# Fancomi2017/InstanceFusion

Hardware: AMD Instinct MI355X
Metric: frames/s + ms/frame (ICP|fuse|instance) at 640x480, 5M surfels, 1/2/4/8 GPU (higher is better)
Workload: dtype f32; 1 GPU; 5000000-surfel map, 640x480 synthetic RGBD stream, 3-level ICP+RGB + surfel fuse + canned-mask instance votes with superpixel refinement; surfels_live=4734799, surfel_slots=4734799, map_order=random, parallelism=replicas x1, loop_frames=90

## Files before the change

instancefusion_amd/csrc/ifx_ctx.h:

```cpp
#pragma once
#include <hip/hip_runtime.h>
#include <stdint.h>
#include <string>
#include <vector>
#include <map>
#include "../../include/ifx_c_api.h"
#include "ifx_dev.h"

#ifndef IFX_LIST_SEGS
#define IFX_LIST_SEGS 8
#endif

struct DevState {
    float pose[16];
    float pose_inv[16];
    float last_pose[16];
    float weighting;
    int dense_enough;
    int count;
    int n_dead;
    int n_new;
    int overflow;
    unsigned int r_max_bits;
    float Rprev[9], tprev[3], Rprev_inv[9];
    float Rcurr[9], tcurr[3];
    double resultRt[16];
    float krkinv[9], kt[3];
    double resultR[9], lastResultR[9];
    float R_lr[9];
    float so3_lastError, so3_lastCount;
    int so3_done;
    float imageBasis[9], kinv[9], krlr[9];
    float lastICPError, lastICPCount, lastRGBError, lastRGBCount, lastSO3Error, lastSO3Count;
    double lastA[36], lastb[6];
    float icp29[29], rgb29[29];
    int rgb_count, rgb_sigma;
    int seg_counts[2];
    int seg_acc[2];
    int fold_total;
    alignas(64) int fold_acc[16][4];
    int first_live;
    int app_count0; unsigned int app_seq0, app_vln0;
    unsigned int result_ticket;
    unsigned int next_seq;
    int hot_stale;
    int range_exceeded;
    float spec_pose[16], spec_pose_inv[16], spec_weighting;
    int skip;
    float lc[24];
    int lc_candidates;
    float vl_pose[16];
    int vl_valid;
    int vl_scan;
    int vl_age;
    int vl_scans;
    unsigned int vl_n[2];
    unsigned int vl_seg_n[2 * IFX_LIST_SEGS], vl_seg_off[2 * IFX_LIST_SEGS];
    long long dbg[8];
    alignas(64) int gn_res[2];
    unsigned int gn_ticket;
    int gn_pad[13];
    double gn_acc[2 * IFX_ACC_REPL * IFX_ACC_STRIDE];
    double gn_acc2[2 * 2 * IFX_ACC_REPL * IFX_ACC_STRIDE];
    alignas(64) int gn_res2[2 * 16];
    alignas(64) unsigned int gn_bar[4 * 32 * 16];
    int gn_timeout;
    int gn_abort;
    int gn_done_seq;
    int gn_spin_limit, gn_fault;
    alignas(64) double gnp_acc[2 * 2 * IFX_ACC_REPL * IFX_ACC_STRIDE];
    alignas(64) int gnp_res[2 * 16];
    alignas(64) double gnp_RRt[2][16];
};

struct IdMap { const uint32_t* seq; int own_n; };
__device__ __forceinline__ int idmap_slot(const IdMap& m, int count, int id)
{
    if (m.own_n <= 0) return (id > 0 && id < count) ? id : -1;
    if (id == 0) return -1;
    int lo = 0, hi = count - 1;
    while (lo <= hi) {
        const int mid = (lo + hi) >> 1;
        const unsigned int v = m.seq[mid];
        if (v == (unsigned int)id) return mid;
        if (v < (unsigned int)id) lo = mid + 1; else hi = mid - 1;
    }
    return -1;
}

struct FrameResult {
// ... 428 lines not shown
```

instancefusion_amd/csrc/ifx_map.hip:

```cpp
#include <climits>
#include "ifx_ctx.h"
#include <string.h>

#define DEAD_TIME (-1.0e9f)
#define ASSOC_NONE 0xFFFFFFFFu
#define ASSOC_NEW 0xFFFFFFFEu
#define MAP_THREADS 256
#ifndef MAP_BLOCKS
#define MAP_BLOCKS 2048
#endif
#ifndef LIST_BLOCKS
#define LIST_BLOCKS 1024
#endif

__device__ inline float get_radius(float depth, float norm_z, float inv_fx, float inv_fy)
{
    float meanFocal = ((1.0f / fabsf(inv_fx)) + (1.0f / fabsf(inv_fy))) / 2.0f;
    const float sqrt2 = 1.41421356237f;
    float radius = (depth / meanFocal) * sqrt2;
    float radius_n = radius / fabsf(norm_z);
    radius_n = fminf(2.0f * radius, radius_n);
    return radius_n;
}
__device__ inline float confidence_fn(float x, float y, float cx, float cy, float weighting)
// ... 1318 lines not shown
        if (T < (float)c.age_epoch) return false;
    }
    return T - wv > 20.f;
}
__global__ void k_vlist_decide(DevState* st, unsigned int* lctr, int force)
{
    if (threadIdx.x != 0) return;
    if (force) st->vl_valid = 0;
    vlist_decide(st);
}

struct VlPlanes { float lx, lz, rx, rz, ty, tz, by, bz; };
__device__ __forceinline__ bool near_frustum(v3 q, float reach, const VlPlanes& P, float maxDepth)
{
    const float len = sqrtf(q.x * q.x + q.y * q.y + q.z * q.z);
    const float D = (reach + VL_TRANS + VL_ROT * (len + reach + VL_TRANS)) * 1.01f + 0.01f;
    if (!(len == len)) return true;
    return !(P.lx * q.x + P.lz * q.z > D || P.rx * q.x + P.rz * q.z > D || P.ty * q.y + P.tz * q.z > D || P.by * q.y + P.bz * q.z > D || -q.z > D || q.z - maxDepth > D);
}
static VlPlanes make_planes(const Cam& c)
{
    VlPlanes P;
    float n = sqrtf(c.fx * c.fx + c.cx * c.cx);
    P.lx = -c.fx / n; P.lz = -c.cx / n;
    n = sqrtf(c.fx * c.fx + (c.cx - c.w) * (c.cx - c.w));
    P.rx = c.fx / n; P.rz = (c.cx - c.w) / n;
    n = sqrtf(c.fy * c.fy + c.cy * c.cy);
    P.ty = -c.fy / n; P.tz = -c.cy / n;
    n = sqrtf(c.fy * c.fy + (c.cy - c.h) * (c.cy - c.h));
    P.by = c.fy / n; P.bz = (c.cy - c.h) / n;
    return P;
}

__global__ __launch_bounds__(MAP_THREADS) void k_cull_frame(DevState* st, const float4* __restrict__ pc_in, float4* __restrict__ pc_rw, float2* __restrict__ tm, Cam c, VlPlanes P,
                                                            int time, unsigned int* __restrict__ list, unsigned int* __restrict__ list_i, Hot* __restrict__ hot, int time_prev)
{
    if (!st->vl_scan) return;
    float Tm[16], T[12];
#pragma unroll
    for (int k = 0; k < 16; k++) Tm[k] = st->vl_pose[k];
    {
        float inv[16];
        pose_inverse(Tm, inv);
#pragma unroll
        for (int k = 0; k < 12; k++) T[k] = inv[k];
    }
    __shared__ BlockCount2 L2;
    if (threadIdx.x == 0) { L2.n[0] = 0; L2.n[1] = 0; }
    __syncthreads();
    const int n = st->count;
    const float reach = __uint_as_float(st->r_max_bits) * 1.41421356f * 1.001f;
    int dead = 0;
    constexpr int CF_ROUNDS = 8, CF_SLOTS = MAP_THREADS * CF_ROUNDS;
    for (int chunk = blockIdx.x; chunk * CF_SLOTS < n; chunk += gridDim.x) {
        unsigned int pos[CF_ROUNDS];
        unsigned int keep = 0, keep_i = 0;
        float4 p4s[CF_ROUNDS];
        float2 ts[CF_ROUNDS];
#pragma unroll
        for (int r = 0; r < CF_ROUNDS; r++) {
            const int i = chunk * CF_SLOTS + r * MAP_THREADS + threadIdx.x;
            const int ii = i < n ? i : n - 1;
            p4s[r] = ld_once(&pc_in[ii]);
            ts[r] = ld_once(&tm[ii]);
        }
        asm volatile("" ::"v"(p4s[0].x), "v"(p4s[1].x), "v"(p4s[2].x), "v"(p4s[3].x), "v"(p4s[4].x), "v"(p4s[5].x), "v"(p4s[6].x), "v"(p4s[7].x), "v"(ts[0].x), "v"(ts[1].x), "v"(ts[2].x),
                     "v"(ts[3].x), "v"(ts[4].x), "v"(ts[5].x), "v"(ts[6].x), "v"(ts[7].x));
#pragma unroll
        for (int r = 0; r < CF_ROUNDS; r++) {
            const int i = chunk * CF_SLOTS + r * MAP_THREADS + threadIdx.x;
            bool in = false, in_i = false;
            if (i < n) {
                const float4 p4 = p4s[r];
                const float2 t = ts[r];
                const float wv = t.y;
                const bool overdue = age_rule_gone(wv, p4.w, time_prev, c) && wv > DEAD_TIME;
                if (overdue) {
                    float4 q4 = p4;
                    q4.w = -1.0f;
                    pc_rw[i] = q4;
                    tm[i] = make_float2(t.x, DEAD_TIME);
                    if (hot) { hot[i].pc = q4; hot[i].tm = make_float2(t.x, DEAD_TIME); }
                    dead++;
                } else if (wv > DEAD_TIME) {
                    in = near_frustum(xf_point(T, v3m(p4.x, p4.y, p4.z)), reach, P, c.maxDepth);
                    if (in && wv > 0.f && (float)time - wv > (float)c.timeDelta) {
                        in = false;
                        in_i = !(p4.w < c.conf);
                    }
                }
            }
            pos[r] = bcount2_reserve(L2, in, in_i);
            keep |= in ? (1u << r) : 0u;
            keep_i |= in_i ? (1u << r) : 0u;
        }
        __syncthreads();
        const int seg = chunk % LIST_SEGS;
        if (threadIdx.x < 2) { L2.base[threadIdx.x] = L2.n[threadIdx.x] ? atomicAdd(list_ctr(c, 1 + threadIdx.x, seg), L2.n[threadIdx.x]) : 0u; L2.n[threadIdx.x] = 0; }
        __syncthreads();
        const unsigned int ba = seg * c.seg_cap + L2.base[0], bi = seg * c.seg_cap + L2.base[1];
#pragma unroll
        for (int r = 0; r < CF_ROUNDS; r++) {
            const unsigned int i = (unsigned int)(chunk * CF_SLOTS + r * MAP_THREADS + threadIdx.x);
            if (keep & (1u << r)) list[ba + pos[r]] = i;
            if (keep_i & (1u << r)) list_i[bi + pos[r]] = i;
        }
    }
    dead = wave_sum_i(dead);
    if ((threadIdx.x & 63) == 0 && dead) atomicAdd(&st->n_dead, dead);
}

__global__ void k_vlist_offsets(DevState* st, Cam c, const float2* __restrict__ tm)
{
    if (!st->vl_scan || threadIdx.x != 0) return;
    for (int which = 0; which < 2; which++) {
        unsigned int run = 0;
        for (int seg = 0; seg < LIST_SEGS; seg++) {
            unsigned int* ctr = list_ctr(c, 1 + which, seg);
            const unsigned int n = *ctr;
            *ctr = 0;
            st->vl_seg_n[which * LIST_SEGS + seg] = n;
            st->vl_seg_off[which * LIST_SEGS + seg] = run;
            run += n;
        }
        st->vl_n[which] = run;
    }
    {
        int f = st->first_live;
        const int n = st->count;
        while (f < n && !(tm[f].y > DEAD_TIME)) f++;
        st->first_live = f;
    }
}
__global__ __launch_bounds__(MAP_THREADS) void k_vlist_concat(const DevState* __restrict__ st, Cam c, const unsigned int* __restrict__ raw_a, const unsigned int* __restrict__ raw_i,
                                                              unsigned int* __restrict__ flat_a, unsigned int* __restrict__ flat_i)
{
    if (!st->vl_scan) return;
    const int which = blockIdx.y, seg = blockIdx.x % LIST_SEGS;
    const unsigned int n = st->vl_seg_n[which * LIST_SEGS + seg], off = st->vl_seg_off[which * LIST_SEGS + seg];
    const unsigned int* __restrict__ raw = (which ? raw_i : raw_a) + (size_t)seg * c.seg_cap;
    unsigned int* __restrict__ flat = (which ? flat_i : flat_a) + off;
    for (unsigned int t = (blockIdx.x / LIST_SEGS) * blockDim.x + threadIdx.x; t < n; t += blockDim.x * (gridDim.x / LIST_SEGS)) flat[t] = raw[t];
}

__global__ __launch_bounds__(MAP_THREADS) void k_index_list(const DevState* __restrict__ st, const float4* __restrict__ pc, const float2* __restrict__ tm, Cam c, int time,
                                                            const unsigned int* __restrict__ list, unsigned long long* __restrict__ keys, const Hot* __restrict__ hot = nullptr)
{
    const int fl = FIRST_LIVE(c);
    float T[12];
#pragma unroll
    for (int k = 0; k < 12; k++) T[k] = st->pose_inv[k];
    const unsigned int n = min(st->vl_n[0], c.seg_cap * LIST_SEGS);
#ifndef INDEX_U
#define INDEX_U 1
#endif
    constexpr int U = INDEX_U;
    const unsigned int stride = blockDim.x * gridDim.x;
    for (unsigned int t = blockIdx.x * blockDim.x + threadIdx.x; t < n; t += U * stride) {
        unsigned int i[U];
        bool in[U];
#pragma unroll
        for (int u = 0; u < U; u++) { const unsigned int tt = t + u * stride; in[u] = tt < n; i[u] = list[in[u] ? tt : t]; }
        float lastT[U];
        float4 p4[U];
#pragma unroll
        for (int u = 0; u < U; u++) { lastT[u] = hot ? hot[i[u]].tm.y : ld_once(&tm[i[u]]).y; p4[u] = hot ? hot[i[u]].pc : ld_once(&pc[i[u]]); }
// ... 1110 lines not shown
{
    age_epoch_begin(h, time);
    h->hot_valid = 0;
    h->last_clean_time = time;
    Cam c = make_cam(h);
    if (part == 0) { c.srank = 0; c.sn = 1; }
    const bool deform = h->graph_nodes > 0 && part != 1;
    if (deform && !h->graph_is_fern) raster_pass(h, d_pose_inv, 0, time - h->cfg.time_delta, LIST_SPLAT, nullptr, false, 0, 1);
    if (part != 2) LAUNCH(h, "cull_clean", dim3(MAP_BLOCKS), dim3(MAP_THREADS), k_cull_clean, h->d_state, d_pose_inv, (const float4*)h->pc, (const float2*)h->tm, c, time, h->key_index,
           h->list_b, h->list_c);
    if (part == 1) return;
    launch_index_resolve(h, d_pose_inv, c, time, INDEX_TAPS, nullptr, nullptr);
    launch_clean_list(h, d_pose_inv, c, time);
    if (deform) {
        LAUNCH_SMEM(h, "deform", dim3(MAP_BLOCKS), dim3(256), (size_t)h->graph_nodes * 64, k_deform, h->d_state, d_pose_inv, h->d_graph, h->graph_nodes, h->graph_is_fern, time, c,
                    (const float4*)h->old_vertex, (float4*)h->pc, (float4*)h->nr, (float2*)h->tm);
        h->graph_nodes = 0;
    }
    launch_new_flags_count(h, d_pose_inv, c, time);
    launch_append_scan(h, c, time, h->own ? (unsigned int*)nullptr : h->list_v);
}

__global__ void k_vlist_invalidate(DevState* st) { if (threadIdx.x == 0) st->vl_valid = 0; }
void hs_invalidate_view(ifx* h) { h->ids_view_ok = 0; LAUNCH(h, "vlist_invalidate", dim3(1), dim3(64), k_vlist_invalidate, h->d_state); }
static void launch_vlist_decide(ifx* h, int force) { LAUNCH(h, "vlist_decide", dim3(1), dim3(64), k_vlist_decide, h->d_state, h->d_list_ctr, force); }
static bool use_view_list(ifx* h) { return h->opt_vlist && h->shard_n <= 1 && !h->own && !h->opt_reference_passes && h->graph_nodes == 0 && !h->view_block && h->tick > 1; }
static bool use_view_list_own(ifx* h) { return h->opt_vlist && h->own && !h->opt_reference_passes && h->graph_nodes == 0 && !h->view_block; }
static void view_scan(ifx* h, int time)
{
    const Cam c = whole_cam(h);
    LAUNCH(h, "cull_frame", dim3(MAP_BLOCKS), dim3(MAP_THREADS), k_cull_frame, h->d_state, (const float4*)h->pc, (float4*)h->pc, (float2*)h->tm, c, make_planes(c), time, h->list_b, h->list_c,
           h->hot_valid ? (Hot*)h->hot : (Hot*)nullptr,
           std::max(0, std::min(time, h->last_clean_time)));
    LAUNCH(h, "vlist_offsets", dim3(1), dim3(64), k_vlist_offsets, h->d_state, c, (const float2*)h->tm);
    LAUNCH(h, "vlist_concat", dim3(256, 2), dim3(MAP_THREADS), k_vlist_concat, (const DevState*)h->d_state, c, h->list_b, h->list_c, h->list_v, h->list_vi);
}
int ifx_vlist_reap(ifx* h)
{
    if (!h->view_dirty) return IFX_OK;
    h->view_dirty = 0;
    h->ids_view_ok = 0;
    launch_vlist_decide(h, 1);
    view_scan(h, h->last_clean_time);
    return IFX_OK;
}
static void index_list_pass(ifx* h, int time, bool taps)
{
    const Cam c = whole_cam(h);
    launch_index_list(h, c, time, (const Hot*)h->frame_hot);
    launch_index_resolve(h, nullptr, c, time, taps ? INDEX_TAPS : INDEX_ASSOC, nullptr, (const Hot*)h->frame_hot);
}

static void view_clean_append(ifx* h, const Cam& c, int time)
{
    h->hot_valid = 0;
    LAUNCH(h, "clean_view", dim3(h->opt_clean_blocks > 0 ? h->opt_clean_blocks : 2 * LIST_BLOCKS), dim3(MAP_THREADS), k_clean_view, h->d_state, c, time, (float4*)h->pc, (const float4*)h->nr, (float2*)h->tm,
           (const float4*)h->index_tap, h->list_v);
    launch_new_flags_count(h, nullptr, c, time);
    launch_append_scan(h, c, time, h->list_v);
}

int ifx_map_frame(ifx* h)
{
    h->clean_raster_pending = 0;
    h->view_frame = 0;
    h->ids_view_ok = 0;
    age_epoch_begin(h, h->tick);
// ... 592 lines not shown
```

instancefusion_amd/csrc/ifx_track.hip:

```cpp
#include "ifx_ctx.h"
#include <math.h>
#include <string.h>


#define BIL_R 6
#define BIL_BX 32
#define BIL_BY 8
template <bool SHIFTED, bool XCLIP>
__device__ __forceinline__ void bil_window(const uint16_t (*tile)[BIL_BX + 2 * BIL_R + 3], const unsigned char* s_mapx, const unsigned char* s_mapy, int x, int y, int bx, int by, int tx1,
                                           int ty1, unsigned int value, float& sum1, float& sum2)
{
    const float ss = 0.024691358f, sc = 0.000555556f;
    constexpr int D = BIL_R * 2 + 1;
    const float fv = (float)value;
    for (int cy = max(y - D / 2, 0); cy < ty1; ++cy) {
        const int ry = SHIFTED ? (int)s_mapy[cy - by + BIL_R + 1] : cy - by + BIL_R + 1;
        const float dy = (float)y - (float)cy, dy2 = dy * dy;
        float tv[D];
#pragma unroll
        for (int q = 0; q < D; q++) {
            const int col = x - D / 2 + q - bx + BIL_R + 1;
            tv[q] = (float)tile[ry][SHIFTED ? (int)s_mapx[col] : col];
        }
#pragma unroll
// ... 184 lines not shown
        v3 r = v3m(qn, qn, qn);
        if (!(u == w - 1 || v == h - 1) && ok00) {
            v3 v01, v10;
            bool ok01 = vert_from_depth(L.depth, w, u + 1, v, L.fx_inv, L.fy_inv, L.cx, L.cy, a.cutoff, v01);
            bool ok10 = vert_from_depth(L.depth, w, u, v + 1, L.fx_inv, L.fy_inv, L.cx, L.cy, a.cutoff, v10);
            if (ok01 && ok10) r = normalized(cross(v01 - v00, v10 - v00));
        }
        L.nmap[v * w + u] = r.x;
        L.nmap[(v + h) * w + u] = r.y;
        L.nmap[(v + 2 * h) * w + u] = r.z;
    }
    {
        const float gsx[9] = {0.52201f, 0.00000f, -0.52201f, 0.79451f, -0.00000f, -0.79451f, 0.52201f, 0.00000f, -0.52201f};
        const float gsy[9] = {0.52201f, 0.79451f, 0.52201f, 0.00000f, 0.00000f, 0.00000f, -0.52201f, -0.79451f, -0.52201f};
        float dxVal = 0, dyVal = 0;
        int k = 8;
        for (int j = max(v - 1, 0); j <= min(v + 1, h - 1); j++)
            for (int i = max(u - 1, 0); i <= min(u + 1, w - 1); i++) {
                dxVal += (float)L.img[j * w + i] * gsx[k];
                dyVal += (float)L.img[j * w + i] * gsy[k];
                --k;
            }
        L.dx[v * w + u] = (int16_t)dxVal;
        L.dy[v * w + u] = (int16_t)dyVal;
    }
}

struct ModelOut {
    float *vcam, *ncam, *depth;
    uint8_t* img;
    float *vprev, *nprev, *cloud;
    float invFx, invFy, cx, cy;
};
__device__ __forceinline__ void model_tail(const DevState* __restrict__ st, int x, int y, int w, int h, v3 vs, v3 ns, float z, const ModelOut& o)
{
    if (o.vprev) {
        const float* P = st->pose;
        const float qn = qnan_f();
        v3 vd = v3m(qn, qn, qn);
        if (!(vs.x != vs.x)) vd = xf_dir(P, vs) + v3m(P[3], P[7], P[11]);
        o.vprev[y * w + x] = vd.x; o.vprev[(y + h) * w + x] = vd.y; o.vprev[(y + 2 * h) * w + x] = vd.z;
        v3 nd = v3m(qn, qn, qn);
        if (!(ns.x != ns.x)) nd = xf_dir(P, ns);
        o.nprev[y * w + x] = nd.x; o.nprev[(y + h) * w + x] = nd.y; o.nprev[(y + 2 * h) * w + x] = nd.z;
    }
    if (o.cloud) {
        o.cloud[(y * w + x) * 3 + 0] = (float)((x - o.cx) * z * o.invFx);
        o.cloud[(y * w + x) * 3 + 1] = (float)((y - o.cy) * z * o.invFy);
        o.cloud[(y * w + x) * 3 + 2] = z;
    }
}
__global__ void k_model_l0(const DevState* __restrict__ st, const float* __restrict__ pv, const float* __restrict__ pn, const uint8_t* __restrict__ pi, const float* __restrict__ fv,
                           const float* __restrict__ fn, const uint8_t* __restrict__ fi, int w, int h, float cutoff, ModelOut o)
{
    int x = blockIdx.x * blockDim.x + threadIdx.x, y = blockIdx.y * blockDim.y + threadIdx.y;
    if (x >= w || y >= h) return;
    const bool fill = fv && !st->dense_enough;
    const float4 v = reinterpret_cast<const float4*>(fill ? fv : pv)[y * w + x];
    const float4 n = reinterpret_cast<const float4*>(fill ? fn : pn)[y * w + x];
    const uint8_t* s = (fill ? fi : pi) + (size_t)(y * w + x) * 4;
    const float qn = qnan_f();
    bool ok = !(v.z == 0);
    v3 vs = v3m(ok ? v.x : qn, ok ? v.y : qn, ok ? v.z : qn), ns = v3m(ok ? n.x : qn, ok ? n.y : qn, ok ? n.z : qn);
    o.vcam[y * w + x] = vs.x; o.vcam[(y + h) * w + x] = vs.y; o.vcam[(y + 2 * h) * w + x] = vs.z;
    o.ncam[y * w + x] = ns.x; o.ncam[(y + h) * w + x] = ns.y; o.ncam[(y + 2 * h) * w + x] = ns.z;
    const float z = (v.z > cutoff || v.z <= 0) ? qn : v.z;
    o.depth[y * w + x] = z;
    o.img[y * w + x] = (uint8_t)(int)((float)s[0] * 0.114f + (float)s[1] * 0.299f + (float)s[2] * 0.587f);
    model_tail(st, x, y, w, h, vs, ns, z, o);
}
struct GnBegin { DevState* st; const DevState* ss; int so3; float fx, fy, cx, cy; int keep_last, enabled, persist; };
__device__ void gn_begin_dev(DevState* st, const DevState* __restrict__ ss, int so3, float fx, float fy, float cx, float cy, int keep_last);
__device__ __forceinline__ void gn_persist_reset(DevState* st, int lt, int nt)
{
    for (int k = lt; k < 2 * 2 * IFX_ACC_REPL * IFX_ACC_STRIDE; k += nt) st->gn_acc2[k] = 0.0;
    if (lt < 32) st->gn_res2[lt] = 0;
    for (int k = lt; k < 4 * 32 * 16; k += nt) st->gn_bar[k] = 0u;
    if (lt == 0) { st->gn_abort = 0; st->gn_done_seq = 0; }
}
__global__ void k_model_down(const DevState* __restrict__ st, const float* __restrict__ vin, const float* __restrict__ nin, const float* __restrict__ din, const uint8_t* __restrict__ iin,
                             int sw, int sh, ModelOut o, GnBegin gb)
{
    if (gb.enabled && blockIdx.x == 0 && blockIdx.y == 0) {
        const int lt = threadIdx.y * blockDim.x + threadIdx.x, nt = blockDim.x * blockDim.y;
        if (gb.persist) gn_persist_reset(gb.st, lt, nt);
        if (lt == 0) gn_begin_dev(gb.st, gb.ss, gb.so3, gb.fx, gb.fy, gb.cx, gb.cy, gb.keep_last);
    }
    const int dw = sw / 2, dh = sh / 2;
    int x = blockIdx.x * blockDim.x + threadIdx.x, y = blockIdx.y * blockDim.y + threadIdx.y;
    if (x >= dw || y >= dh) return;
    const float qn = qnan_f();
    const int xs = x * 2, ys = y * 2;
    v3 res[2];
#pragma unroll
    for (int m = 0; m < 2; m++) {
        const float* in = m ? nin : vin;
        float* out = m ? o.ncam : o.vcam;
        float x00 = in[ys * sw + xs], x01 = in[ys * sw + xs + 1], x10 = in[(ys + 1) * sw + xs], x11 = in[(ys + 1) * sw + xs + 1];
        v3 n = v3m(qn, qn, qn);
        if (!((x00 != x00) || (x01 != x01) || (x10 != x10) || (x11 != x11))) {
            n.x = (x00 + x01 + x10 + x11) / 4;
            const float* py = in + sh * sw;
// ... 1705 lines not shown
                for (int k = 0; k < 9; k++) { st->Rcurr[k] = Rc[k]; st->krkinv[k] = krkn[k]; }
#pragma unroll
                for (int k = 0; k < 3; k++) { st->tcurr[k] = tcn[k]; st->kt[k] = ktn[k]; }
                if (a.final_level) track_end_vals(st, RGB, 1, Rc, tcn, Rp, tpv, a.weight_mult, a.commit, a.lctr);
                st->gn_done_seq = a.level + 1;
            }
        }
        __syncthreads();
    }
    (void)failed;
}


__global__ void k_commit_pose(DevState* st, unsigned int* lctr)
{
    (void)lctr;
    const int t = threadIdx.x;
    float cp = 0.f;
    if (t < 16) cp = st->spec_pose[t]; else if (t < 32) cp = st->spec_pose_inv[t - 16]; else if (t == 32) cp = st->spec_weighting;
    float A[16], B[16];
    int valid = 0, age = 0;
    if (t == 0) {
#pragma unroll
        for (int k = 0; k < 16; k++) { A[k] = st->vl_pose[k]; B[k] = st->spec_pose[k]; }
        valid = st->vl_valid; age = st->vl_age;
    }
    if (t < 16) st->pose[t] = cp; else if (t < 32) st->pose_inv[t - 16] = cp; else if (t == 32) st->weighting = cp;
    if (t != 0) return;
    vlist_decide_core(st, A, B, valid, age);
}



static const dim3 B2(32, 8);
static inline dim3 G2(int w, int h) { return dim3(cdiv(w, 32), cdiv(h, 8)); }

int ifx_alloc_tracker(ifx* h)
{
    Pyr& p = h->pyr;
    for (int i = 0; i < IFX_NUM_PYRS; i++) {
        p.w[i] = h->w >> i; p.h[i] = h->h >> i;
        size_t n = (size_t)p.w[i] * p.h[i];
        for (int q = 0; q < 2; q++) {
            FrameSlot& f = h->slot[q];
            HIPCHK(h, hipMalloc(&f.depth_tmp[i], n * 2));
            HIPCHK(h, hipMalloc(&f.vmap_curr[i], n * 12)); HIPCHK(h, hipMalloc(&f.nmap_curr[i], n * 12));
            HIPCHK(h, hipMalloc(&f.next_img[i], n)); HIPCHK(h, hipMemset(f.next_img[i], 0, n));
            HIPCHK(h, hipMalloc(&f.didx[i], n * 2)); HIPCHK(h, hipMalloc(&f.didy[i], n * 2));
        }
        HIPCHK(h, hipMalloc(&p.vmap_cam[i], n * 12)); HIPCHK(h, hipMalloc(&p.nmap_cam[i], n * 12));
        HIPCHK(h, hipMalloc(&p.vmap_prev[i], n * 12)); HIPCHK(h, hipMalloc(&p.nmap_prev[i], n * 12));
        HIPCHK(h, hipMalloc(&p.last_depth[i], n * 4));
        HIPCHK(h, hipMalloc(&p.last_img[i], n));
        HIPCHK(h, hipMalloc(&p.cloud[i], n * 12));
        HIPCHK(h, hipMalloc(&p.corres[i], n * 8));
    }
    const int maxb = 1024;
    HIPCHK(h, hipMalloc(&p.acc, (3 * IFX_ACC_REPL * IFX_ACC_STRIDE * sizeof(double))));
    HIPCHK(h, hipMemset(p.acc, 0, (3 * IFX_ACC_REPL * IFX_ACC_STRIDE * sizeof(double))));
    {
        int cus = 0, dev = 0;
        hipGetDevice(&dev);
        hipDeviceGetAttribute(&cus, hipDeviceAttributeMultiprocessorCount, dev);
        int occ[4] = {0, 0, 0, 0};
        hipOccupancyMaxActiveBlocksPerMultiprocessor(&occ[0], k_gn_level<1>, RED_THREADS, 0);
        hipOccupancyMaxActiveBlocksPerMultiprocessor(&occ[1], k_gn_level<2>, RED_THREADS, 0);
// ... 59 lines not shown
static inline int red_blocks(ifx* h, int n, int it = RED_IT)
{
    int b = cdiv(n, RED_THREADS * it);
    const int cap = h->opt_icp_blocks > 0 ? h->opt_icp_blocks : std::max(456, std::min(1024, h->P / 2048));
    if (b > cap) b = cap;
    if (b < 1) b = 1;
    return b;
}

int ifx_tracker_init_first(ifx* h)
{
    Pyr& p = h->pyr;
    LAUNCH(h, "intensity", dim3(cdiv(h->P, 256)), dim3(256), k_intensity, h->rgb, 3, h->P, p.lastnext_img[0]);
    for (int i = 0; i + 1 < IFX_NUM_PYRS; i++)
        LAUNCH(h, "pyrdown_u8", G2(p.w[i + 1], p.h[i + 1]), B2, k_pyrdown_gauss_u8, p.lastnext_img[i], p.w[i], p.h[i], p.lastnext_img[i + 1]);
    return IFX_OK;
}

static inline GnBegin gb_none() { GnBegin g; g.st = nullptr; g.ss = nullptr; g.so3 = 0; g.fx = g.fy = g.cx = g.cy = 0.f; g.keep_last = 0; g.enabled = 0; g.persist = 0; return g; }
static void tracker_init_model(ifx* h, DevState* st, Pyr& p, float icp_weight, const float* pv, const float* pn, const uint8_t* pi, const float* fv, const float* fn, const uint8_t* fi, const GnBegin* gbp = nullptr)
{
    const GnBegin gb_off = gb_none();
    const ifx_config& c = h->cfg;
    const int rgb = icp_weight < 100;
    const int iterations[3] = {c.fast_odom ? 3 : 10, c.pyramid ? 5 : 0, c.pyramid ? 4 : 0};
    ModelOut o3[IFX_NUM_PYRS];
    for (int i = 0; i < IFX_NUM_PYRS; i++) {
        const float div = (float)(1 << i);
        ModelOut& o = o3[i];
        o.vcam = p.vmap_cam[i]; o.ncam = p.nmap_cam[i]; o.depth = p.last_depth[i]; o.img = p.last_img[i];
        o.vprev = p.vmap_prev[i]; o.nprev = p.nmap_prev[i]; o.cloud = (rgb && iterations[i] > 0) ? p.cloud[i] : nullptr;
        o.invFx = 1.0f / (c.fx / div); o.invFy = 1.0f / (c.fy / div); o.cx = c.cx / div; o.cy = c.cy / div;
    }
    for (int i = 0; i < IFX_NUM_PYRS; i++) {
        const ModelOut& o = o3[i];
        if (i == 0) LAUNCH(h, "model_l0", G2(h->w, h->h), B2, k_model_l0, st, pv, pn, pi, fv, fn, fi, h->w, h->h, 6.0f, o);
        else LAUNCH(h, "model_down", G2(p.w[i], p.h[i]), B2, k_model_down, st, p.vmap_cam[i - 1], p.nmap_cam[i - 1], p.last_depth[i - 1], p.last_img[i - 1], p.w[i - 1], p.h[i - 1], o, (i == IFX_NUM_PYRS - 1 && gbp) ? *gbp : gb_off);
    }
}

__global__ void k_sobel(const uint8_t* __restrict__ img, int w, int h, int16_t* __restrict__ dx, int16_t* __restrict__ dy)
{
    const int u = blockIdx.x * blockDim.x + threadIdx.x, v = blockIdx.y * blockDim.y + threadIdx.y;
    if (u >= w || v >= h) return;
    const float gsx[9] = {0.52201f, 0.00000f, -0.52201f, 0.79451f, -0.00000f, -0.79451f, 0.52201f, 0.00000f, -0.52201f};
    const float gsy[9] = {0.52201f, 0.79451f, 0.52201f, 0.00000f, 0.00000f, 0.00000f, -0.52201f, -0.79451f, -0.52201f};
    float dxVal = 0, dyVal = 0;
    int k = 8;
    for (int j = max(v - 1, 0); j <= min(v + 1, h - 1); j++)
        for (int i = max(u - 1, 0); i <= min(u + 1, w - 1); i++) {
            dxVal += (float)img[j * w + i] * gsx[k];
            dyVal += (float)img[j * w + i] * gsy[k];
            --k;
        }
    dx[v * w + u] = (int16_t)dxVal;
    dy[v * w + u] = (int16_t)dyVal;
}
static void tracker_init_frame_maps(ifx* h, DevState* st, Pyr& p, const float* pv, const float* pn, const uint8_t* pi)
{
    for (int i = 0; i < IFX_NUM_PYRS; i++) {
        ModelOut o;
        o.vcam = p.vmap_curr[i]; o.ncam = p.nmap_curr[i]; o.depth = p.next_depth[i]; o.img = p.next_img[i];
        o.vprev = nullptr; o.nprev = nullptr; o.cloud = nullptr;
        o.invFx = 0; o.invFy = 0; o.cx = 0; o.cy = 0;
        if (i == 0) LAUNCH(h, "model_l0", G2(h->w, h->h), B2, k_model_l0, st, pv, pn, pi, (const float*)nullptr, (const float*)nullptr, (const uint8_t*)nullptr, h->w, h->h, 6.0f, o);
        else LAUNCH(h, "model_down", G2(p.w[i], p.h[i]), B2, k_model_down, st, p.vmap_curr[i - 1], p.nmap_curr[i - 1], p.next_depth[i - 1], p.next_img[i - 1], p.w[i - 1], p.h[i - 1], o, gb_none());
        LAUNCH(h, "sobel", G2(p.w[i], p.h[i]), B2, k_sobel, p.next_img[i], p.w[i], p.h[i], p.didx[i], p.didy[i]);
    }
}

static void tracker_init_frame(ifx* h, const uint16_t* depth_filt, const uint8_t* rgb)
{
    Pyr& p = h->pyr;
    (void)depth_filt;
    LAUNCH(h, "intensity", dim3(cdiv(h->P, 256)), dim3(256), k_intensity, rgb, 3, h->P, p.next_img[0]);
    for (int i = 1; i < IFX_NUM_PYRS; i++)
        LAUNCH(h, "frame_down", G2(p.w[i], p.h[i]), B2, k_frame_down, p.depth_tmp[i - 1], p.next_img[i - 1], p.w[i - 1], p.h[i - 1], p.depth_tmp[i], p.next_img[i]);
    FrameLevels fl;
    int blocks = 0;
    for (int i = 0; i < IFX_NUM_PYRS; i++) {
        float div = (float)(1 << i);
        float fx = h->cfg.fx / div, fy = h->cfg.fy / div;
        FrameLevel& L = fl.l[i];
        L.depth = p.depth_tmp[i]; L.img = p.next_img[i]; L.vmap = p.vmap_curr[i]; L.nmap = p.nmap_curr[i]; L.dx = p.didx[i]; L.dy = p.didy[i];
        L.w = p.w[i]; L.h = p.h[i]; L.tiles_x = cdiv(p.w[i], 32); L.first_block = blocks;
        L.fx_inv = 1.f / fx; L.fy_inv = 1.f / fy; L.cx = h->cfg.cx / div; L.cy = h->cfg.cy / div;
        blocks += L.tiles_x * cdiv(p.h[i], 8);
    }
    fl.cutoff = h->cfg.max_depth_processed;
    LAUNCH(h, "frame_maps", dim3(blocks), dim3(256), k_frame_maps, fl);
}

int ifx_comm_ready(ifx* h);
int ifx_comm_allreduce_f64(ifx* h, double* d_ptr, int n);
static inline const char* icp_name_rows(int level) { static const char* const n[3] = {"icp_residual_rows@L0", "icp_residual_rows@L1", "icp_residual_rows@L2"}; return n[level]; }
static void tracker_run(ifx* h, DevState* st, Pyr& p, float icp_weight, int so3, float weight_mult, int commit, bool frame_tracker, int keep_last = 0)
{
    const ifx_config& c = h->cfg;
    const int icp = icp_weight > 0, rgb = icp_weight < 100;
    int iterations[3] = {c.fast_odom ? 3 : 10, c.pyramid ? 5 : 0, c.pyramid ? 4 : 0};
    int first = -1;
// ... 703 lines not shown
```

Before: 1634 frames/s.

## Fuse vlist offsets into cull tail and merge model levels 0 and 1

Result: no change. 1643 frames/s (median of 4 runs) (+0.6%).

```diff
diff --git a/instancefusion_amd/csrc/ifx_ctx.h b/instancefusion_amd/csrc/ifx_ctx.h
--- a/instancefusion_amd/csrc/ifx_ctx.h
+++ b/instancefusion_amd/csrc/ifx_ctx.h
@@ -56,6 +56,8 @@
     int vl_scans;
     unsigned int vl_n[2];
     unsigned int vl_seg_n[2 * IFX_LIST_SEGS], vl_seg_off[2 * IFX_LIST_SEGS];
+    alignas(64) unsigned int vl_ticket;
+    int vl_pad[15];
     long long dbg[8];
     alignas(64) int gn_res[2];
     unsigned int gn_ticket;
diff --git a/instancefusion_amd/csrc/ifx_map.hip b/instancefusion_amd/csrc/ifx_map.hip
--- a/instancefusion_amd/csrc/ifx_map.hip
+++ b/instancefusion_amd/csrc/ifx_map.hip
@@ -1374,6 +1374,26 @@
     return P;
 }
 
+__device__ __forceinline__ void vlist_offsets_dev(DevState* st, const Cam& c, const float2* tm, int n)
+{
+    for (int which = 0; which < 2; which++) {
+        unsigned int run = 0;
+        for (int seg = 0; seg < LIST_SEGS; seg++) {
+            unsigned int* ctr = list_ctr(c, 1 + which, seg);
+            const unsigned int m = __hip_atomic_load(ctr, __ATOMIC_RELAXED, __HIP_MEMORY_SCOPE_AGENT);
+            __hip_atomic_store(ctr, 0u, __ATOMIC_RELAXED, __HIP_MEMORY_SCOPE_AGENT);
+            st->vl_seg_n[which * LIST_SEGS + seg] = m;
+            st->vl_seg_off[which * LIST_SEGS + seg] = run;
+            run += m;
+        }
+        st->vl_n[which] = run;
+    }
+    {
+        int f = st->first_live;
+        while (f < n && !(__hip_atomic_load(&tm[f].y, __ATOMIC_RELAXED, __HIP_MEMORY_SCOPE_AGENT) > DEAD_TIME)) f++;
+        st->first_live = f;
+    }
+}
 __global__ __launch_bounds__(MAP_THREADS) void k_cull_frame(DevState* st, const float4* __restrict__ pc_in, float4* __restrict__ pc_rw, float2* __restrict__ tm, Cam c, VlPlanes P,
                                                             int time, unsigned int* __restrict__ list, unsigned int* __restrict__ list_i, Hot* __restrict__ hot, int time_prev)
 {
@@ -1421,7 +1441,7 @@
                     float4 q4 = p4;
                     q4.w = -1.0f;
                     pc_rw[i] = q4;
-                    tm[i] = make_float2(t.x, DEAD_TIME);
+                    __hip_atomic_store(&tm[i].y, DEAD_TIME, __ATOMIC_RELAXED, __HIP_MEMORY_SCOPE_AGENT);
                     if (hot) { hot[i].pc = q4; hot[i].tm = make_float2(t.x, DEAD_TIME); }
                     dead++;
                 } else if (wv > DEAD_TIME) {
@@ -1450,30 +1470,19 @@
     }
     dead = wave_sum_i(dead);
     if ((threadIdx.x & 63) == 0 && dead) atomicAdd(&st->n_dead, dead);
-}
-
-__global__ void k_vlist_offsets(DevState* st, Cam c, const float2* __restrict__ tm)
-{
-    if (!st->vl_scan || threadIdx.x != 0) return;
-    for (int which = 0; which < 2; which++) {
-        unsigned int run = 0;
-        for (int seg = 0; seg < LIST_SEGS; seg++) {
-            unsigned int* ctr = list_ctr(c, 1 + which, seg);
-            const unsigned int n = *ctr;
-            *ctr = 0;
-            st->vl_seg_n[which * LIST_SEGS + seg] = n;
-            st->vl_seg_off[which * LIST_SEGS + seg] = run;
-            run += n;
-        }
-        st->vl_n[which] = run;
-    }
-    {
-        int f = st->first_live;
-        const int n = st->count;
-        while (f < n && !(tm[f].y > DEAD_TIME)) f++;
-        st->first_live = f;
-    }
-}
+    __shared__ int s_last;
+    asm volatile("s_waitcnt vmcnt(0)" ::: "memory");
+    __syncthreads();
+    if (threadIdx.x == 0) {
+        const unsigned int t = __hip_atomic_fetch_add(&st->vl_ticket, 1u, __ATOMIC_RELAXED, __HIP_MEMORY_SCOPE_AGENT);
+        s_last = (t == gridDim.x - 1u);
+    }
+    __syncthreads();
+    if (!s_last || threadIdx.x != 0) return;
+    __hip_atomic_store(&st->vl_ticket, 0u, __ATOMIC_RELAXED, __HIP_MEMORY_SCOPE_AGENT);
+    vlist_offsets_dev(st, c, tm, n);
+}
+
 __global__ __launch_bounds__(MAP_THREADS) void k_vlist_concat(const DevState* __restrict__ st, Cam c, const unsigned int* __restrict__ raw_a, const unsigned int* __restrict__ raw_i,
                                                               unsigned int* __restrict__ flat_a, unsigned int* __restrict__ flat_i)
 {
@@ -2650,7 +2659,6 @@
     LAUNCH(h, "cull_frame", dim3(MAP_BLOCKS), dim3(MAP_THREADS), k_cull_frame, h->d_state, (const float4*)h->pc, (float4*)h->pc, (float2*)h->tm, c, make_planes(c), time, h->list_b, h->list_c,
            h->hot_valid ? (Hot*)h->hot : (Hot*)nullptr,
            std::max(0, std::min(time, h->last_clean_time)));
-    LAUNCH(h, "vlist_offsets", dim3(1), dim3(64), k_vlist_offsets, h->d_state, c, (const float2*)h->tm);
     LAUNCH(h, "vlist_concat", dim3(256, 2), dim3(MAP_THREADS), k_vlist_concat, (const DevState*)h->d_state, c, h->list_b, h->list_c, h->list_v, h->list_vi);
 }
 int ifx_vlist_reap(ifx* h)
diff --git a/instancefusion_amd/csrc/ifx_track.hip b/instancefusion_amd/csrc/ifx_track.hip
--- a/instancefusion_amd/csrc/ifx_track.hip
+++ b/instancefusion_amd/csrc/ifx_track.hip
@@ -240,42 +240,131 @@
     float *vprev, *nprev, *cloud;
     float invFx, invFy, cx, cy;
 };
-__device__ __forceinline__ void model_tail(const DevState* __restrict__ st, int x, int y, int w, int h, v3 vs, v3 ns, float z, const ModelOut& o)
-{
+__device__ __forceinline__ void model_tail_vals(const DevState* __restrict__ st, int x, int y, v3 vs, v3 ns, float z, const ModelOut& o, v3& vd, v3& nd, v3& cl)
+{
+    const float qn = qnan_f();
+    vd = v3m(qn, qn, qn); nd = v3m(qn, qn, qn); cl = v3m(qn, qn, qn);
     if (o.vprev) {
         const float* P = st->pose;
-        const float qn = qnan_f();
-        v3 vd = v3m(qn, qn, qn);
         if (!(vs.x != vs.x)) vd = xf_dir(P, vs) + v3m(P[3], P[7], P[11]);
+        if (!(ns.x != ns.x)) nd = xf_dir(P, ns);
+    }
+    if (o.cloud) cl = v3m((float)((x - o.cx) * z * o.invFx), (float)((y - o.cy) * z * o.invFy), z);
+}
+__device__ __forceinline__ void model_tail(const DevState* __restrict__ st, int x, int y, int w, int h, v3 vs, v3 ns, float z, const ModelOut& o)
+{
+    v3 vd, nd, cl;
+    model_tail_vals(st, x, y, vs, ns, z, o, vd, nd, cl);
+    if (o.vprev) {
         o.vprev[y * w + x] = vd.x; o.vprev[(y + h) * w + x] = vd.y; o.vprev[(y + 2 * h) * w + x] = vd.z;
-        v3 nd = v3m(qn, qn, qn);
-        if (!(ns.x != ns.x)) nd = xf_dir(P, ns);
         o.nprev[y * w + x] = nd.x; o.nprev[(y + h) * w + x] = nd.y; o.nprev[(y + 2 * h) * w + x] = nd.z;
     }
     if (o.cloud) {
-        o.cloud[(y * w + x) * 3 + 0] = (float)((x - o.cx) * z * o.invFx);
-        o.cloud[(y * w + x) * 3 + 1] = (float)((y - o.cy) * z * o.invFy);
-        o.cloud[(y * w + x) * 3 + 2] = z;
-    }
-}
-__global__ void k_model_l0(const DevState* __restrict__ st, const float* __restrict__ pv, const float* __restrict__ pn, const uint8_t* __restrict__ pi, const float* __restrict__ fv,
-                           const float* __restrict__ fn, const uint8_t* __restrict__ fi, int w, int h, float cutoff, ModelOut o)
-{
-    int x = blockIdx.x * blockDim.x + threadIdx.x, y = blockIdx.y * blockDim.y + threadIdx.y;
-    if (x >= w || y >= h) return;
+        o.cloud[(y * w + x) * 3 + 0] = cl.x;
+        o.cloud[(y * w + x) * 3 + 1] = cl.y;
+        o.cloud[(y * w + x) * 3 + 2] = cl.z;
+    }
+}
+#define ML_TW 68
+#define ML_TH 20
+__device__ __forceinline__ void st_pair(float* p, float a, float b) { *reinterpret_cast<float2*>(p) = make_float2(a, b); }
+__global__ __launch_bounds__(256) void k_model_l0(const DevState* __restrict__ st, const float* __restrict__ pv, const float* __restrict__ pn, const uint8_t* __restrict__ pi,
+                                                   const float* __restrict__ fv, const float* __restrict__ fn, const uint8_t* __restrict__ fi, int w, int h, float cutoff, ModelOut o0,
+                                                   ModelOut o1)
+{
+    __shared__ float s_z[ML_TH][ML_TW];
+    __shared__ uint8_t s_i[ML_TH][ML_TW];
     const bool fill = fv && !st->dense_enough;
-    const float4 v = reinterpret_cast<const float4*>(fill ? fv : pv)[y * w + x];
-    const float4 n = reinterpret_cast<const float4*>(fill ? fn : pn)[y * w + x];
-    const uint8_t* s = (fill ? fi : pi) + (size_t)(y * w + x) * 4;
+    const float4* __restrict__ sv = reinterpret_cast<const float4*>(fill ? fv : pv);
+    const float4* __restrict__ sn = reinterpret_cast<const float4*>(fill ? fn : pn);
+    const uint8_t* __restrict__ si = fill ? fi : pi;
+    const int dw = w / 2, dh = h / 2;
+    const int x = blockIdx.x * 32 + threadIdx.x, y = blockIdx.y * 8 + threadIdx.y;
+    const int ox = blockIdx.x * 64 - 2, oy = blockIdx.y * 16 - 2;
     const float qn = qnan_f();
-    bool ok = !(v.z == 0);
-    v3 vs = v3m(ok ? v.x : qn, ok ? v.y : qn, ok ? v.z : qn), ns = v3m(ok ? n.x : qn, ok ? n.y : qn, ok ? n.z : qn);
-    o.vcam[y * w + x] = vs.x; o.vcam[(y + h) * w + x] = vs.y; o.vcam[(y + 2 * h) * w + x] = vs.z;
-    o.ncam[y * w + x] = ns.x; o.ncam[(y + h) * w + x] = ns.y; o.ncam[(y + 2 * h) * w + x] = ns.z;
-    const float z = (v.z > cutoff || v.z <= 0) ? qn : v.z;
-    o.depth[y * w + x] = z;
-    o.img[y * w + x] = (uint8_t)(int)((float)s[0] * 0.114f + (float)s[1] * 0.299f + (float)s[2] * 0.587f);
-    model_tail(st, x, y, w, h, vs, ns, z, o);
+    const bool mine = x < dw && y < dh;
+    v3 vs[2][2], ns[2][2];
+    if (mine) {
+#pragma unroll
+        for (int dy = 0; dy < 2; dy++) {
+            const int py = 2 * y + dy, px = 2 * x;
+            float z[2];
+            uint8_t in[2];
+            v3 vd[2], nd[2], cl[2];
+#pragma unroll
+            for (int dx = 0; dx < 2; dx++) {
+                const float4 v = sv[py * w + px + dx];
+                const float4 n = sn[py * w + px + dx];
+                const uint8_t* s = si + (size_t)(py * w + px + dx) * 4;
+                const bool ok = !(v.z == 0);
+                vs[dy][dx] = v3m(ok ? v.x : qn, ok ? v.y : qn, ok ? v.z : qn);
+                ns[dy][dx] = v3m(ok ? n.x : qn, ok ? n.y : qn, ok ? n.z : qn);
+                z[dx] = (v.z > cutoff || v.z <= 0) ? qn : v.z;
+                in[dx] = (uint8_t)(int)((float)s[0] * 0.114f + (float)s[1] * 0.299f + (float)s[2] * 0.587f);
+                model_tail_vals(st, px + dx, py, vs[dy][dx], ns[dy][dx], z[dx], o0, vd[dx], nd[dx], cl[dx]);
+                s_z[py - oy][px + dx - ox] = z[dx];
+                s_i[py - oy][px + dx - ox] = in[dx];
+            }
+            const int i0 = py * w + px, i1 = (py + h) * w + px, i2 = (py + 2 * h) * w + px;
+            st_pair(o0.vcam + i0, vs[dy][0].x, vs[dy][1].x); st_pair(o0.vcam + i1, vs[dy][0].y, vs[dy][1].y); st_pair(o0.vcam + i2, vs[dy][0].z, vs[dy][1].z);
+            st_pair(o0.ncam + i0, ns[dy][0].x, ns[dy][1].x); st_pair(o0.ncam + i1, ns[dy][0].y, ns[dy][1].y); st_pair(o0.ncam + i2, ns[dy][0].z, ns[dy][1].z);
+            st_pair(o0.depth + i0, z[0], z[1]);
+            *reinterpret_cast<uchar2*>(o0.img + i0) = make_uchar2(in[0], in[1]);
+            if (o0.vprev) {
+                st_pair(o0.vprev + i0, vd[0].x, vd[1].x); st_pair(o0.vprev + i1, vd[0].y, vd[1].y); st_pair(o0.vprev + i2, vd[0].z, vd[1].z);
+                st_pair(o0.nprev + i0, nd[0].x, nd[1].x); st_pair(o0.nprev + i1, nd[0].y, nd[1].y); st_pair(o0.nprev + i2, nd[0].z, nd[1].z);
+            }
+            if (o0.cloud) {
+                st_pair(o0.cloud + i0 * 3, cl[0].x, cl[0].y); st_pair(o0.cloud + i0 * 3 + 2, cl[0].z, cl[1].x); st_pair(o0.cloud + i0 * 3 + 4, cl[1].y, cl[1].z);
+            }
+        }
+    }
+    for (int e = threadIdx.y * 32 + threadIdx.x; e < 4 * ML_TW + 4 * 16; e += 256) {
+        int r, cidx;
+        if (e < 4 * ML_TW) { r = e / ML_TW; cidx = e - r * ML_TW; if (r >= 2) r += 16; }
+        else { const int k = e - 4 * ML_TW; r = 2 + (k >> 2); cidx = k & 3; if (cidx >= 2) cidx += 64; }
+        const int gx = ox + cidx, gy = oy + r;
+        if (gx >= 0 && gx < w && gy >= 0 && gy < h) {
+            const float vz = sv[gy * w + gx].z;
+            const uint8_t* s = si + (size_t)(gy * w + gx) * 4;
+            s_z[r][cidx] = (vz > cutoff || vz <= 0) ? qn : vz;
+            s_i[r][cidx] = (uint8_t)(int)((float)s[0] * 0.114f + (float)s[1] * 0.299f + (float)s[2] * 0.587f);
+        }
+    }
+    __syncthreads();
+    if (!mine) return;
+    v3 res[2];
+#pragma unroll
+    for (int m = 0; m < 2; m++) {
+        const v3(&q)[2][2] = m ? ns : vs;
+        float* out = m ? o1.ncam : o1.vcam;
+        const float x00 = q[0][0].x, x01 = q[0][1].x, x10 = q[1][0].x, x11 = q[1][1].x;
+        v3 n = v3m(qn, qn, qn);
+        if (!((x00 != x00) || (x01 != x01) || (x10 != x10) || (x11 != x11))) {
+            n.x = (x00 + x01 + x10 + x11) / 4;
+            n.y = (q[0][0].y + q[0][1].y + q[1][0].y + q[1][1].y) / 4;
+            n.z = (q[0][0].z + q[0][1].z + q[1][0].z + q[1][1].z) / 4;
+            if (m) n = normalized(n);
+        }
+        out[y * dw + x] = n.x; out[(y + dh) * dw + x] = n.y; out[(y + 2 * dh) * dw + x] = n.z;
+        res[m] = n;
+    }
+    const int D = 5, sw = w, sh = h;
+    const int tx = min(2 * x - D / 2 + D, sw - 1), ty = min(2 * y - D / 2 + D, sh - 1);
+    float sumf = 0, sumi = 0;
+    int cntf = 0, cnti = 0;
+    for (int cy = max(0, 2 * y - D / 2); cy < ty; ++cy)
+        for (int cx = max(0, 2 * x - D / 2); cx < tx; ++cx) {
+            const float g = c_gauss25[(ty - cy - 1) * 5 + (tx - cx - 1)];
+            const float sf = s_z[cy - oy][cx - ox];
+            if (!(sf != sf)) { sumf += sf * g; cntf += (int)g; }
+            const int si_ = s_i[cy - oy][cx - ox];
+            if (si_ > 0) { sumi += si_ * g; cnti += (int)g; }
+        }
+    const float z = (float)(sumf / (float)cntf);
+    o1.depth[y * dw + x] = z;
+    o1.img[y * dw + x] = cnti ? (uint8_t)f2i_rz(sumi / (float)cnti) : (uint8_t)0;
+    model_tail(st, x, y, dw, dh, res[0], res[1], z, o1);
 }
 struct GnBegin { DevState* st; const DevState* ss; int so3; float fx, fy, cx, cy; int keep_last, enabled, persist; };
 __device__ void gn_begin_dev(DevState* st, const DevState* __restrict__ ss, int so3, float fx, float fy, float cx, float cy, int keep_last);
@@ -2047,6 +2136,7 @@
 
 
 
+
 static const dim3 B2(32, 8);
 static inline dim3 G2(int w, int h) { return dim3(cdiv(w, 32), cdiv(h, 8)); }
 
@@ -2172,11 +2262,9 @@
         o.vprev = p.vmap_prev[i]; o.nprev = p.nmap_prev[i]; o.cloud = (rgb && iterations[i] > 0) ? p.cloud[i] : nullptr;
         o.invFx = 1.0f / (c.fx / div); o.invFy = 1.0f / (c.fy / div); o.cx = c.cx / div; o.cy = c.cy / div;
     }
-    for (int i = 0; i < IFX_NUM_PYRS; i++) {
-        const ModelOut& o = o3[i];
-        if (i == 0) LAUNCH(h, "model_l0", G2(h->w, h->h), B2, k_model_l0, st, pv, pn, pi, fv, fn, fi, h->w, h->h, 6.0f, o);
-        else LAUNCH(h, "model_down", G2(p.w[i], p.h[i]), B2, k_model_down, st, p.vmap_cam[i - 1], p.nmap_cam[i - 1], p.last_depth[i - 1], p.last_img[i - 1], p.w[i - 1], p.h[i - 1], o, (i == IFX_NUM_PYRS - 1 && gbp) ? *gbp : gb_off);
-    }
+    static_assert(IFX_NUM_PYRS == 3, "levels 0 and 1 share a launch");
+    LAUNCH(h, "model_l0", G2(p.w[1], p.h[1]), B2, k_model_l0, st, pv, pn, pi, fv, fn, fi, h->w, h->h, 6.0f, o3[0], o3[1]);
+    LAUNCH(h, "model_down", G2(p.w[2], p.h[2]), B2, k_model_down, st, p.vmap_cam[1], p.nmap_cam[1], p.last_depth[1], p.last_img[1], p.w[1], p.h[1], o3[2], gbp ? *gbp : gb_off);
 }
 
 __global__ void k_sobel(const uint8_t* __restrict__ img, int w, int h, int16_t* __restrict__ dx, int16_t* __restrict__ dy)
@@ -2198,15 +2286,17 @@
 }
 static void tracker_init_frame_maps(ifx* h, DevState* st, Pyr& p, const float* pv, const float* pn, const uint8_t* pi)
 {
+    ModelOut o3[IFX_NUM_PYRS];
     for (int i = 0; i < IFX_NUM_PYRS; i++) {
-        ModelOut o;
+        ModelOut& o = o3[i];
         o.vcam = p.vmap_curr[i]; o.ncam = p.nmap_curr[i]; o.depth = p.next_depth[i]; o.img = p.next_img[i];
         o.vprev = nullptr; o.nprev = nullptr; o.cloud = nullptr;
         o.invFx = 0; o.invFy = 0; o.cx = 0; o.cy = 0;
-        if (i == 0) LAUNCH(h, "model_l0", G2(h->w, h->h), B2, k_model_l0, st, pv, pn, pi, (const float*)nullptr, (const float*)nullptr, (const uint8_t*)nullptr, h->w, h->h, 6.0f, o);
-        else LAUNCH(h, "model_down", G2(p.w[i], p.h[i]), B2, k_model_down, st, p.vmap_curr[i - 1], p.nmap_curr[i - 1], p.next_depth[i - 1], p.next_img[i - 1], p.w[i - 1], p.h[i - 1], o, gb_none());
-        LAUNCH(h, "sobel", G2(p.w[i], p.h[i]), B2, k_sobel, p.next_img[i], p.w[i], p.h[i], p.didx[i], p.didy[i]);
-    }
+    }
+    static_assert(IFX_NUM_PYRS == 3, "levels 0 and 1 share a launch");
+    LAUNCH(h, "model_l0", G2(p.w[1], p.h[1]), B2, k_model_l0, st, pv, pn, pi, (const float*)nullptr, (const float*)nullptr, (const uint8_t*)nullptr, h->w, h->h, 6.0f, o3[0], o3[1]);
+    LAUNCH(h, "model_down", G2(p.w[2], p.h[2]), B2, k_model_down, st, p.vmap_curr[1], p.nmap_curr[1], p.next_depth[1], p.next_img[1], p.w[1], p.h[1], o3[2], gb_none());
+    for (int i = 0; i < IFX_NUM_PYRS; i++) LAUNCH(h, "sobel", G2(p.w[i], p.h[i]), B2, k_sobel, p.next_img[i], p.w[i], p.h[i], p.didx[i], p.didy[i]);
 }
 
 static void tracker_init_frame(ifx* h, const uint16_t* depth_filt, const uint8_t* rgb)
```
